# daducci/AMICO

Measured on AMD Instinct MI355X. Metric: voxels/sec (whole node), NODDI fit, higher is better.
Workload: dtype f64; 1 GPU; NODDI fit, 1000000 masked voxels per GPU, 99-volume 2-shell scheme (9 b0 + 30@b700 + 60@b2000), 145 atoms, ndirs=500, inputs resident in HBM; voxels_per_gpu=1000000, global_voxels=1000000, parallelism=voxel shards x1, one RCCL all_gather of the maps per step

## Files before the change

amico_amd/csrc/amx_kernels.hpp:

```cpp
#pragma once
#include <type_traits>
#include "amx_solver.hpp"
#include "amx_gram_solver.hpp"

namespace amx {

struct Chunk { int dir, start, count, pad; };
constexpr int kSeedKD = 12;
constexpr int kAuxU = 0, kAuxU2 = 12, kAuxB0 = 24, kAuxYY = 25, kAuxYB = 26, kAuxTmin = 27, kAuxN = 28;
__host__ __device__ constexpr int gemm_rows(int n_atoms) { return ((n_atoms + kAuxN + 15) / 16) * 16; }
constexpr int kScreenLd = 192;

enum StatusSlot { ST_ERRVOX = 0, ST_II1 = 1, ST_II2 = 2, ST_OVERFLOW = 3, ST_ITCAP = 4, ST_RERUN = 5, ST_GUARD = 6, ST_GUARDVOX = 7, ST_EXACT = 8, ST_GRAM = 11, ST_ITERS = 14, ST_SEED = 17, ST_LEFT = 92, ST_CLIP = 95, ST_ERRPACK = 96, ST_ERRKIND = 98, ST_WORDS = 100 };

struct FitCommon {
    const void *tiles;
    const double *y;
    const float *y32;
    const int *perm;
    const Chunk *chunks;
    const int *n_chunks;
    const int *list;
    const int *list_count;
    const int *lutidx;
// ... 208 lines not shown
        st_ = S.solve(As, ldA, nS, n_atoms, yr, rowok, scl, allowed, kLasso ? a.c.lam1 : 0.0, kLasso ? a.c.lam2 : 0.0, rs, rl, lane, gdir, a.ldG, seed, scr);
    }
    const int st = __builtin_amdgcn_readfirstlane(st_);
    if (st == kOverflow) {
        if (lane == 0) {
            const int k = atomicAdd(a.c.ovf_count, 1);
            a.c.ovf_list[k] = (STAGE == 4 && a.list_is_pos) ? pos : vox;
        }
    } else {
    if (st == kIterCap && lane == 0) atomicAdd(&a.c.status[ST_ITCAP], 1);
    if (st > kIterCap && lane == 0) { atomicAdd(&a.c.status[ST_GUARD], 1); a.c.status[ST_GUARDVOX] = vox * 8 + st; }
#ifdef AMX_PHASES
    if constexpr (STAGE == 1 || STAGE == 3) {
        if (lane == 0 && S.seeded == 1) {
            unsigned long long *acc = reinterpret_cast<unsigned long long *>(const_cast<int *>(a.c.n_chunks) + 16) + (STAGE == 1 ? 0 : 8);
            for (int k = 0; k < 8; k++) atomicAdd(&acc[k], (unsigned long long)S.ph[k]);
        }
    }
#endif
#ifdef AMX_STATS
    if (lane == 0) { constexpr int sx = kLasso ? 1 : STAGE - 1; atomicAdd(&a.c.status[ST_EXACT + sx], S.n_exact); atomicAdd(&a.c.status[ST_GRAM + sx], S.n_gram); atomicAdd(&a.c.status[ST_ITERS + sx], S.iters);
        if constexpr (STAGE == 4) { if (S.seeded >= 0) atomicAdd(&a.c.status[ST_SEED + 18], 1); if (S.seeded == 1) atomicAdd(&a.c.status[ST_SEED + 19], 1); }
        if constexpr (!kLasso) { if (S.seeded >= 0) atomicAdd(&a.c.status[ST_SEED + (STAGE == 1 ? 0 : 2)], 1); if (S.seeded == 1) atomicAdd(&a.c.status[ST_SEED + (STAGE == 1 ? 1 : 3)], 1); if (S.seeded == 0 && STAGE == 1) atomicAdd(&a.c.status[ST_SEED + 6 + S.seed_why], 1); } }
#endif
    const bool act = lane < S.np;
    if (a.c.xdbg) {
        constexpr int row = (STAGE == 1) ? 0 : (kLasso ? 1 : 2);
        double *dst = a.c.xdbg + ((size_t)vox * 3 + row) * n_atoms;
        store_x_dense<NQ>(dst, n_atoms, lane, S.np, S.idx, S.x);
        if (kLasso && lane == 0) {
            asm volatile("s_waitcnt vmcnt(0)" ::: "memory");
            dst[iso_atom] = a.xiso[(size_t)vox * 2];
            if (dot_atom >= 0) dst[dot_atom] = a.xiso[(size_t)vox * 2 + 1];
        }
    }

    if constexpr (STAGE == 1) {
        const unsigned long long mi = ballot64(act && S.idx == iso_atom), md = ballot64(act && S.idx == dot_atom);
        const double xi = mi ? bcast(S.x, __builtin_ctzll(mi)) : 0.0;
        const double xd = md ? bcast(S.x, __builtin_ctzll(md)) : 0.0;
        if (lane == 0) { a.xiso[(size_t)vox * 2] = xi; a.xiso[(size_t)vox * 2 + 1] = xd; }
    } else if constexpr (kLasso) {
        if (lane < 4) wmask[lane] = 0ull;
        if (act && S.x > 0.0) atomicOr(&wmask[S.idx >> 6], 1ull << (S.idx & 63));
        if (lane < 4) a.supp[(size_t)vox * 4 + lane] = wmask[lane];
    } else {
        double rsq = 0.0, ysq = 0.0;
        if (a.c.flags & 3u) {
            S.residual(yr, 0.0);
#pragma unroll
            for (int rr = 0; rr < NR; rr++) { rsq += S.r[rr] * S.r[rr]; ysq += yr[rr] * yr[rr]; }
            rsq = wave_sum(rsq); ysq = wave_sum(ysq);
        }
        const double xs = act ? S.x : 0.0;
        const bool iswm = act && S.idx < n_wm;
        const double sum_atoms = wave_sum(xs) + 1e-16;
        const double sum_wm = wave_sum(iswm ? xs / sum_atoms : 0.0) + 1e-16;
        double f1 = 0.0, f2 = 0.0, k1 = 0.0;
        if (iswm) {
            const float ic = a.icvf[S.idx];
            const double t = xs / sum_atoms / sum_wm;
            f1 = (double)ic * t;
            f2 = (double)((float)(1.0 - (double)ic)) * t;
            k1 = (double)a.kappa[S.idx] * t;
        }
        f1 = wave_sum(f1); f2 = wave_sum(f2); k1 = wave_sum(k1);
        const double ndi = f1 / (f1 + f2 + 1e-16);
        const double odi = odi_from_kappa(k1);
        const double fwf = wave_sum((act && S.idx == iso_atom) ? xs : 0.0) / sum_atoms;
        const double dot = wave_sum((act && S.idx == dot_atom) ? xs : 0.0) / sum_atoms;
        if (lane == 0) {
            double *e = a.est + (size_t)vox * a.n_maps;
            e[0] = ndi; e[1] = odi; e[2] = fwf;
            if (a.is_exvivo) e[3] = dot;
            if (a.rmse) a.rmse[vox] = sqrt(rsq / (double)nS);
            if (a.nrmse) a.nrmse[vox] = (ysq > 1e-16) ? sqrt(rsq / ysq) : 0.0;
            if (a.mod) { const double tf = 1.0 - fwf; a.mod[(size_t)vox * 2] = ndi * tf; a.mod[(size_t)vox * 2 + 1] = odi * tf; }
        }
    }
    }
    }
}

struct FwArgs {
    FitCommon c;
    int n_perp, n_iso, is_mouse, n_maps;
    double *est, *rmse, *nrmse, *ycorr;
    double *cproj;
    const double *prep;
    unsigned *p0;
    int ldC;
    int *queue;
    int sub_per_chunk;
};

template <int NR, int NQ, int MAXP>
__device__ __forceinline__ void fw_voxel(const FwArgs &a, const float *As, double *rs, double *rl, int vox, int lane)
{
    const int nS = a.c.nS, ldA = a.c.ldA, n_atoms = a.c.n_atoms, n_perp = a.n_perp;
    double yr[NR];
    const bool ok = load_rows<NR>(a.c, vox, nS, lane, yr);
    bool rowok[NR];
    double scl[NQ];
    unsigned long long allowed[NQ];
#pragma unroll
    for (int rr = 0; rr < NR; rr++) rowok[rr] = (lane + kWave * rr) < nS;
#pragma unroll
    for (int q = 0; q < NQ; q++) {
        const int cnt = n_atoms - kWave * q;
        allowed[q] = cnt >= 64 ? ~0ull : (cnt > 0 ? ((1ull << cnt) - 1ull) : 0ull);
        scl[q] = 1.0;
    }
    if (!ok) {
        if (lane < a.n_maps) a.est[(size_t)vox * a.n_maps + lane] = __builtin_nan("");
        if (lane == 0 && a.rmse) a.rmse[vox] = __builtin_nan("");
        if (lane == 0 && a.nrmse) a.nrmse[vox] = __builtin_nan("");
        if (a.ycorr)
            for (int i = lane; i < nS; i += kWave) a.ycorr[(size_t)vox * nS + i] = __builtin_nan("");
    }
    if (ok) {
    NNSolver<NR, NQ, MAXP, true, float> S;
    const int st = __builtin_amdgcn_readfirstlane(S.solve(As, ldA, nS, n_atoms, yr, rowok, scl, allowed, a.c.lam1, a.c.lam2, rs, rl, lane));
    if (st == kOverflow) {
        if (lane == 0) { const int k = atomicAdd(a.c.ovf_count, 1); a.c.ovf_list[k] = vox; }
    } else {
    if (st == kIterCap && lane == 0) atomicAdd(&a.c.status[ST_ITCAP], 1);
    if (st > kIterCap && lane == 0) { atomicAdd(&a.c.status[ST_GUARD], 1); a.c.status[ST_GUARDVOX] = vox * 8 + st; }
    const bool act = lane < S.np;
    const double xs = act ? S.x : 0.0;
    if (a.c.xdbg) store_x_dense<NQ>(a.c.xdbg + (size_t)vox * n_atoms, n_atoms, lane, S.np, S.idx, S.x);
    const double x_sum = wave_sum(xs) + 1e-16;
    const double v = wave_sum((act && S.idx < n_perp) ? xs : 0.0) / x_sum;
    const double vb = wave_sum((act && S.idx == n_perp) ? xs : 0.0) / x_sum;
    const double vc = wave_sum((act && S.idx == n_perp + 1) ? xs : 0.0) / x_sum;
    double rsq = 0.0, ysq = 0.0;
#pragma unroll
    for (int rr = 0; rr < NR; rr++) { rsq += S.r[rr] * S.r[rr]; ysq += yr[rr] * yr[rr]; }
    if (a.c.flags & 3u) { rsq = wave_sum(rsq); ysq = wave_sum(ysq); }
    if (lane == 0) {
        double *e = a.est + (size_t)vox * a.n_maps;
        e[0] = v; e[1] = 1.0 - v;
        if (a.is_mouse) { e[2] = vb; e[3] = vc; }
        if (a.rmse) a.rmse[vox] = sqrt(rsq / (double)nS);
        if (a.nrmse) a.nrmse[vox] = (ysq > 1e-16) ? sqrt(rsq / ysq) : 0.0;
    }
    if (a.ycorr) {
        double fw[NR];
#pragma unroll
        for (int rr = 0; rr < NR; rr++) fw[rr] = 0.0;
        for (int s = 0; s < S.np; s++) {
            const int at = bcast_i(S.idx, s);
            if (at >= n_perp) {
                const double xv = bcast(S.x, s);
#pragma unroll
                for (int rr = 0; rr < NR; rr++) {
                    const int i = lane + kWave * rr;
                    if (i < nS) fw[rr] += (double)As[i * ldA + at] * xv;
                }
            }
        }
#pragma unroll
        for (int rr = 0; rr < NR; rr++) {
            const int i = lane + kWave * rr;
            if (i < nS) { const double yc = yr[rr] - fw[rr]; a.ycorr[(size_t)vox * nS + i] = yc < 0.0 ? 0.0 : yc; }
        }
    }
// ... 105 lines not shown
    unsigned long long allowed[NQ];
#pragma unroll
    for (int rr = 0; rr < NR; rr++) rowok[rr] = (lane + kWave * rr) < nS;
#pragma unroll
    for (int q = 0; q < NQ; q++) {
        const int cnt = n_atoms - kWave * q;
        allowed[q] = cnt >= 64 ? ~0ull : (cnt > 0 ? ((1ull << cnt) - 1ull) : 0ull);
        scl[q] = 1.0;
    }
    if (!ok) {
        if (lane < 3) a.est[(size_t)vox * 3 + lane] = __builtin_nan("");
        if (lane == 0 && a.rmse) a.rmse[vox] = __builtin_nan("");
        if (lane == 0 && a.nrmse) a.nrmse[vox] = __builtin_nan("");
    }
    if (ok) {
    typename std::conditional<QR, NNSolver<NR, NQ, MAXP, true, float>, GramSolver<NR, NQ, MAXP, float>>::type S;
    const bool dense = NQ == 1 && n_atoms <= MAXP && a.c.lam2 >= 1e-2 && !(a.c.flags & 0x80000000u);
    int st_;
    if constexpr (QR) {
        st_ = S.solve(As, ldA, nS, n_atoms, yr, rowok, scl, allowed, a.c.lam1, a.c.lam2, rs, rl, lane);
    } else if constexpr (NQ == 1) {
        st_ = dense ? S.solve_dense(As, ldA, nS, n_atoms, yr, a.c.lam1, a.c.lam2, rs, rl, lane, gdir, a.ldG, Lf, lf_inv)
                    : S.solve(As, ldA, nS, n_atoms, yr, rowok, scl, allowed, a.c.lam1, a.c.lam2, rs, rl, lane, gdir, a.ldG);
    } else {
        st_ = S.solve(As, ldA, nS, n_atoms, yr, rowok, scl, allowed, a.c.lam1, a.c.lam2, rs, rl, lane, gdir, a.ldG);
    }
    const int st = __builtin_amdgcn_readfirstlane(st_);
    if (st == kOverflow) {
        if (lane == 0) { const int k = atomicAdd(a.c.ovf_count, 1); a.c.ovf_list[k] = vox; }
    } else {
    if (st == kIterCap && lane == 0) atomicAdd(&a.c.status[ST_ITCAP], 1);
    if (st > kIterCap && lane == 0) { atomicAdd(&a.c.status[ST_GUARD], 1); a.c.status[ST_GUARDVOX] = vox * 8 + st; }
    const bool act = lane < S.np;
    const int at = act ? S.idx : 0;
    const double xs = act ? S.x : 0.0;
    if (a.c.xdbg) store_x_dense<NQ>(a.c.xdbg + (size_t)vox * n_atoms, n_atoms, lane, S.np, S.idx, xs);
    double f1 = wave_sum((act && at < n_rs) ? xs : 0.0);
    const double f2 = wave_sum((act && at >= n_rs && at < n_rs + n_perp) ? xs : 0.0) + 1e-16;
    const double v = f1 / (f1 + f2 + 1e-16);
    f1 += 1e-16;
    double am = wave_sum((act && at < n_rs) ? a.Rs[at] * xs : 0.0);
    am = 1e6 * 2.0 * am / f1;
    const double d = (4.0 * v) / (3.14159265358979323846 * (am * am) + 1e-16);
    if (lane == 0) { double *e = a.est + (size_t)vox * 3; e[0] = v; e[1] = am; e[2] = d; }
    if (a.c.flags & 3u) {
        double est[NR];
#pragma unroll
        for (int rr = 0; rr < NR; rr++) est[rr] = 0.0;
        for (int s = 0; s < S.np; s++) {
            const int as = bcast_i(S.idx, s);
            const double xv = bcast(xs, s);
#pragma unroll
            for (int rr = 0; rr < NR; rr++) {
                const int i = lane + kWave * rr;
                if (i < nS) est[rr] += (double)As[i * ldA + as] * xv;
            }
        }
        double rsq = 0.0, ysq = 0.0;
#pragma unroll
        for (int rr = 0; rr < NR; rr++) { const double t = yr[rr] - est[rr]; rsq += t * t; ysq += yr[rr] * yr[rr]; }
        rsq = wave_sum(rsq); ysq = wave_sum(ysq);
        if (lane == 0) {
            if (a.rmse) a.rmse[vox] = sqrt(rsq / (double)nS);
            if (a.nrmse) a.nrmse[vox] = (ysq > 1e-16) ? sqrt(rsq / ysq) : 0.0;
        }
    }
    }
    }
}

__host__ __device__ constexpr int solver_lds_words(bool gram, int maxp, bool ridge = true)
{
    return gram ? (maxp + 1) * (maxp + 2) : (ridge ? 2 : 1) * (maxp + 1) * (maxp + 1);
}

__device__ __forceinline__ int xcd_chunk(int b, int n_chunks)
{
    const int per = (n_chunks + 7) >> 3;
    const int cid = (b & 7) * per + (b >> 3);
    return ((b >> 3) < per && cid < n_chunks) ? cid : -1;
}


__device__ __forceinline__ int next_ticket(unsigned *ticket, int lane)
{
    const unsigned off = (unsigned)(uintptr_t)ticket;
    const unsigned inc = lane == 0 ? 1u : 0u;
    unsigned old;
    asm volatile("ds_add_rtn_u32 %0, %1, %2\n\ts_waitcnt lgkmcnt(0)" : "=v"(old) : "v"(off), "v"(inc) : "memory");
    return __builtin_amdgcn_readfirstlane((int)old);
}

#define AMX_KERNEL_PROLOGUE_GT(AT, NRv, NQv, NWv, RLWv, GTv)                                                \
    extern __shared__ __attribute__((aligned(16))) unsigned char smem[];                              \
    const int lane = threadIdx.x & 63, wave = threadIdx.x >> 6;                                       \
    const int words = a.c.nS * a.c.ldA;                                                               \
    const int words_pad = (GTv) ? 0 : ((words + kWave * NQv + 3) & ~3);                               \
    AT *As = reinterpret_cast<AT *>(smem);                                                            \
    double *rs_all = reinterpret_cast<double *>(smem + (((size_t)words_pad * sizeof(AT) + 15) & ~(size_t)15)); \
    double *rs = rs_all + wave * (NRv * kWave);                                                       \
    const int nw_ = (int)blockDim.x >> 6;                     \
    double *rl_all = rs_all + nw_ * NRv * kWave;                                                      \
    double *rl = rl_all + wave * (RLWv);                                                              \
    unsigned long long *wm_all = reinterpret_cast<unsigned long long *>(rl_all + nw_ * (RLWv)); \
    unsigned long long *wmask = wm_all + wave * 4;                                                    \

#define AMX_KERNEL_PROLOGUE(AT, NRv, NQv, NWv, RLWv) AMX_KERNEL_PROLOGUE_GT(AT, NRv, NQv, NWv, RLWv, false)
constexpr int kTileSlack = 512;

template <int STAGE, int NR, int NQ, int MAXP, int NW, bool LIST, typename AT = float, bool GT = false>
__global__ void __launch_bounds__(NW * 64, (NW <= 4 && !LIST && !GT) ? 2 : 1) k_noddi(const NoddiArgs a)
{
    static_assert(!GT || std::is_same<AT, float>::value, "the global tile is the float32 dictionary itself");
    using ATs = typename std::conditional<GT, gtile<float>, AT>::type;
    constexpr int RLW = solver_lds_words(STAGE == 4, MAXP, STAGE == 2);
    AMX_KERNEL_PROLOGUE_GT(AT, NR, NQ, NW, RLW, GT)
    const float *tiles = reinterpret_cast<const float *>(a.c.tiles);
    if (!LIST) {
        const int cid = xcd_chunk((int)blockIdx.x, *a.c.n_chunks);
        if (cid < 0) return;
        const Chunk ck = a.c.chunks[cid];
        unsigned *ticket = reinterpret_cast<unsigned *>(wm_all + nw_ * 4);
        if ((STAGE == 1 || STAGE == 3 || STAGE == 4) && a.rlist != nullptr) {
            const int left = a.rcount[cid];
            if (left == 0) return;
            if (threadIdx.x == 0) atomicAdd(&a.c.status[ST_LEFT + (STAGE == 1 ? 0 : (STAGE == 3 ? 2 : 1))], left);
        }
        if (threadIdx.x == 0) { ticket[0] = (unsigned)nw_; ticket[1] = (unsigned)nw_; }
        const AT *At = As;
        if constexpr (GT) At = reinterpret_cast<const AT *>(tiles + (size_t)ck.dir * a.c.tile_stride);
        else stage_noddi_tile<AT>(As, tiles + (size_t)ck.dir * a.c.tile_stride, words, words_pad - words);
        float *Sf = nullptr;
        if ((STAGE == 1 || STAGE == 3) && a.scr_S != nullptr && a.seeds != nullptr) {
            Sf = reinterpret_cast<float *>(ticket + 4);
            const float *src = a.scr_S + (size_t)ck.dir * kSeedKD * kScreenLd;
            for (int e = threadIdx.x; e < kSeedKD * kScreenLd; e += blockDim.x) Sf[e] = src[e];
        }
        if (STAGE == 4 && a.scr2_S != nullptr && a.seeds2 != nullptr) {
            Sf = reinterpret_cast<float *>(ticket + 4);
            const float *src = a.scr2_S + (size_t)ck.dir * kSeedKD * kScreenLd;
            for (int e = threadIdx.x; e < kSeedKD * kScreenLd; e += blockDim.x) Sf[e] = src[e];
        }
        __syncthreads();
#ifdef AMX_STATIC_VOXELS
        for (int k = wave; k < ck.count; k += nw_) {
            noddi_voxel<STAGE, NR, NQ, MAXP, ATs>(a, reinterpret_cast<const ATs *>(At), rs, rl, wmask, a.c.perm[ck.start + k], ck.dir, lane);
        }
#else
        if ((STAGE == 1 || STAGE == 3 || STAGE == 4) && a.rlist != nullptr) {
            const int cnt = a.rcount[cid];
            const bool two = (STAGE == 1 || STAGE == 3) && a.done != nullptr;
            for (int pass = 0; pass < (two ? 2 : 1); pass++) {
                unsigned *tk = ticket + pass;
                for (int k = wave; k < cnt; k = next_ticket(tk, lane)) {
                    const int pos = a.rlist[ck.start + k];
                    if (two) {
                        const int flag = __builtin_amdgcn_readfirstlane((int)a.done[pos]);
                        if ((flag == 2) != (pass == 1)) continue;
                    }
                    noddi_voxel<STAGE, NR, NQ, MAXP, ATs>(a, reinterpret_cast<const ATs *>(At), rs, rl, wmask, a.c.perm[pos], ck.dir, lane, pos, Sf);
                }
            }
        } else {
            for (int k = wave; k < ck.count; k = next_ticket(ticket, lane)) {
                noddi_voxel<STAGE, NR, NQ, MAXP, ATs>(a, reinterpret_cast<const ATs *>(At), rs, rl, wmask, a.c.perm[ck.start + k], ck.dir, lane, ck.start + k, Sf);
            }
        }
#endif
    } else {
        const int cnt = *a.c.list_count;
        for (int it = blockIdx.x; it < cnt; it += gridDim.x) {
            const int e = a.c.list[it];
            const int pos = (STAGE == 4 && a.list_is_pos) ? e : -1;
            const int vox = (STAGE == 4 && a.list_is_pos) ? a.c.perm[e] : e;
            if constexpr (GT) {
                noddi_voxel<STAGE, NR, NQ, MAXP, ATs>(a, reinterpret_cast<const ATs *>(tiles + (size_t)a.c.lutidx[vox] * a.c.tile_stride), rs, rl, wmask, vox, a.c.lutidx[vox], lane, pos);
            } else {
                __syncthreads();
                stage_noddi_tile<AT>(As, tiles + (size_t)a.c.lutidx[vox] * a.c.tile_stride, words, words_pad - words);
                __syncthreads();
                noddi_voxel<STAGE, NR, NQ, MAXP, AT>(a, As, rs, rl, wmask, vox, a.c.lutidx[vox], lane, pos);
            }
        }
    }
}

template <int NR, int NQ, int MAXP, int NW, bool LIST>
__global__ void __launch_bounds__(NW * 64) k_freewater(const FwArgs a)
{
    AMX_KERNEL_PROLOGUE(float, NR, NQ, NW, solver_lds_words(false, MAXP))
    (void)wmask;
    const float *tiles = reinterpret_cast<const float *>(a.c.tiles);
    if (!LIST) {
        const int cid = xcd_chunk((int)blockIdx.x, *a.c.n_chunks);
        if (cid < 0) return;
        const Chunk ck = a.c.chunks[cid];
        unsigned *ticket = reinterpret_cast<unsigned *>(wm_all + nw_ * 4);
        if (threadIdx.x == 0) *ticket = (unsigned)nw_;
        stage_tile<float>(As, tiles + (size_t)ck.dir * a.c.tile_stride, words, words_pad - words);
        __syncthreads();
        for (int k = wave; k < ck.count; k = next_ticket(ticket, lane)) {
            fw_voxel<NR, NQ, MAXP>(a, As, rs, rl, a.c.perm[ck.start + k], lane);
        }
    } else {
        const int cnt = *a.c.list_count;
        for (int it = blockIdx.x; it < cnt; it += gridDim.x) {
            const int vox = a.c.list[it];
            __syncthreads();
            stage_tile<float>(As, tiles + (size_t)a.c.lutidx[vox] * a.c.tile_stride, words, words_pad - words);
            __syncthreads();
            fw_voxel<NR, NQ, MAXP>(a, As, rs, rl, vox, lane);
        }
    }
}

template <int NR, int NQ, int MAXP, int NW, bool LIST>
__global__ void __launch_bounds__(NW * 64) k_sandi(const SandiArgs a)
{
    AMX_KERNEL_PROLOGUE(double, NR, NQ, NW, solver_lds_words(false, MAXP))
    (void)wmask;
    const double *tiles = reinterpret_cast<const double *>(a.c.tiles);
    if (!LIST) {
        const int cid = xcd_chunk((int)blockIdx.x, *a.c.n_chunks);
        if (cid < 0) return;
        const Chunk ck = a.c.chunks[cid];
        unsigned *ticket = reinterpret_cast<unsigned *>(wm_all + nw_ * 4);
        if (threadIdx.x == 0) *ticket = (unsigned)nw_;
        stage_tile<double>(As, tiles, words, words_pad - words);
        __syncthreads();
        for (int k = wave; k < ck.count; k = next_ticket(ticket, lane)) {
            sandi_voxel<NR, NQ, MAXP>(a, As, rs, rl, a.c.perm[ck.start + k], lane);
        }
    } else {
        const int cnt = *a.c.list_count;
        stage_tile<double>(As, tiles, words, words_pad - words);
        __syncthreads();
// ... 169 lines not shown
```

amico_amd/csrc/amx_solver.hpp:

```cpp
#pragma once
#include <hip/hip_runtime.h>
#include <stdint.h>

namespace amx {

constexpr int kWave = 64;

#ifdef AMX_PHASES
#define AMX_PH(k) do { const long long t__ = (long long)__builtin_readcyclecounter(); ph[k] += t__ - pht; pht = t__; } while (0)
#else
#define AMX_PH(k) do { } while (0)
#endif
enum SolveStatus : int { kSolved = 0, kOverflow = 1, kIterCap = 2, kGuardSelect = 3, kGuardOuter = 4 };
struct SeedScreen {
    const float *Sf = nullptr;
    int ld = 0;
    double kappa = 0.0;
    const double *ytil = nullptr;
    const double *Sg = nullptr;
    int *count = nullptr;
};
constexpr unsigned long long kSeedNone = ~0ull;

__device__ __forceinline__ double bcast(double v, int l)
{
    int lo = __builtin_amdgcn_readlane(__double2loint(v), l);
    int hi = __builtin_amdgcn_readlane(__double2hiint(v), l);
    return __hiloint2double(hi, lo);
}
__device__ __forceinline__ int bcast_i(int v, int l) { return __builtin_amdgcn_readlane(v, l); }

template <int CTRL, int ROWM, int BANKM>
__device__ __forceinline__ double dpp_move(double v, double ident)
{
    int lo = __builtin_amdgcn_update_dpp(__double2loint(ident), __double2loint(v), CTRL, ROWM, BANKM, false);
    int hi = __builtin_amdgcn_update_dpp(__double2hiint(ident), __double2hiint(v), CTRL, ROWM, BANKM, false);
    return __hiloint2double(hi, lo);
}
template <int CTRL>
__device__ __forceinline__ double dpp_zero(double v)
{
    int lo = __builtin_amdgcn_update_dpp(0, __double2loint(v), CTRL, 0xf, 0xf, true);
    int hi = __builtin_amdgcn_update_dpp(0, __double2hiint(v), CTRL, 0xf, 0xf, true);
    return __hiloint2double(hi, lo);
}
#define AMX_ROW_SWAP(BUILTIN, k, A, B)                                                                             \
    do {                                                                                                           \
        const auto lo_ = BUILTIN((unsigned)__double2loint(k), (unsigned)__double2loint(k), false, false);          \
        const auto hi_ = BUILTIN((unsigned)__double2hiint(k), (unsigned)__double2hiint(k), false, false);          \
        A = __hiloint2double((int)hi_[0], (int)lo_[0]); B = __hiloint2double((int)hi_[1], (int)lo_[1]);            \
    } while (0)
__device__ __forceinline__ double rows_allreduce(double k)
{
    double a, b;
    AMX_ROW_SWAP(__builtin_amdgcn_permlane16_swap, k, a, b); k = a + b;
    AMX_ROW_SWAP(__builtin_amdgcn_permlane32_swap, k, a, b); k = a + b;
    return k;
}
__device__ __forceinline__ double wave_sum(double v)
{
    double t = v + dpp_zero<0xB1>(v);
    t += dpp_zero<0x4E>(t);
    t += dpp_zero<0x141>(t);
    t += dpp_zero<0x140>(t);
    return rows_allreduce(t);
}
__device__ __forceinline__ double wave_max(double v)
{
    double t = fmax(v, dpp_zero<0xB1>(v));
    t = fmax(t, dpp_zero<0x4E>(t));
    t = fmax(t, dpp_zero<0x141>(t));
    t = fmax(t, dpp_zero<0x140>(t));
    double a, b;
    AMX_ROW_SWAP(__builtin_amdgcn_permlane16_swap, t, a, b); t = fmax(a, b);
    AMX_ROW_SWAP(__builtin_amdgcn_permlane32_swap, t, a, b); t = fmax(a, b);
    return t;
}
__device__ __forceinline__ double wave_min(double v) { return -wave_max(-v); }
__device__ __forceinline__ double rows_allmax(double k)
{
    double a, b;
    AMX_ROW_SWAP(__builtin_amdgcn_permlane16_swap, k, a, b); k = fmax(a, b);
    AMX_ROW_SWAP(__builtin_amdgcn_permlane32_swap, k, a, b); k = fmax(a, b);
    return k;
}
// ... 722 lines not shown
                } else {
                    AMX_PH(3);
                    const int kn = np;
#pragma unroll
                    for (int m = 0; m < MAXP; m++) {
                        if (m == kn) {
#pragma unroll
                            for (int rr = 0; rr < NR; rr++) Q[m][rr] = v[rr] * binv;
                        }
                    }
                    if (lane <= kn) Rl[lane * LDR + kn] = (lane == kn) ? beta : rho;
                    if (RIDGE && lane <= kn) Ql[lane * LDR + kn] = va * binv;
                    if (lane == kn) { d = dnew; e = enew; rinv = binv; x = 0.0; sc = sct; idx = t; }
                    fl &= 0xff00ffffu; cyc_banned = false;
                    if (lane == tl) fl |= 0x100u << tq;
                    np = kn + 1;
                    last_added = t;
                    added = true;

                }
            }
            if (redo) continue;
            if (!added) {
                if (status == kSolved && cyc_banned && second_looks < 3) {
                    fl &= 0xff00ffffu; cyc_banned = false; second_looks++; force_exact = true; last_added = -1;
                    continue;
                }
                break;
            }

            AMX_PH(4);
            for (bool feasible = false; !feasible && status == kSolved;) {
                if (++iters > itmax) { status = kIterCap; break; }
                double rhs = d - lam1 * e;
                {
                    const int li = (lane < MAXP ? lane : MAXP - 1) * LDR;
                    for (int j = np - 1; j >= 0; j--) {
                        const double col = Rl[li + j];
                        const double zj = bcast(rhs * rinv, j);
                        if (lane < j) rhs -= col * zj;
                    }
                }
                const double z = (lane < np) ? rhs * rinv : 0.0;
                const bool act = lane < np;
                const bool neg = act && !(z > 0.0);
                AMX_PH(5);
                const bool any = ballot64(neg) != 0ull;
                unsigned long long rem = 0ull;
                if (any) {
                    const double den = x - z;
                    const double ratio = neg ? ((den > 0.0) ? x / den : 0.0) : inf;
                    const double alpha = wave_min(ratio);
                    const unsigned long long hit = ballot64(neg && ratio == alpha);
                    const int kmin = hit ? __builtin_ctzll(hit) : -1;
                    x = act ? x + alpha * (z - x) : 0.0;
                    if (lane == kmin) x = 0.0;
                    rem = ballot64(act && !(x > 0.0));
                } else {
                    x = act ? z : 0.0;
                }
                for (int guard = 0; rem != 0ull && guard < kWave; ++guard) {
                    const int k = 63 - __builtin_clzll(rem);
                    rem &= ~(1ull << k);
                    const int a = bcast_i(idx, k);
                    if (a == last_added) { cyc_banned = true; if (lane == (a & 63)) fl |= 0x10000u << (a >> 6); }
                    if (G != nullptr) {
                        const double dl = -bcast(sc * xprev, k);
                        const double *gc = G + (size_t)a * ldG + lane;
#pragma unroll
                        for (int q = 0; q < NQ; q++) u[q] -= gc[kWave * q] * dl;
                    }
                    if (lane == (a & 63)) fl &= ~(0x1000000u << (a >> 6));
                    remove_slot(k, lane, fl);
                }
                if (np == 0) x = 0.0;
                feasible = !any || np == 0;
                AMX_PH(6);
            }
        }
        return status;
    }
};

}
```

Baseline: 156.0 million voxels/s.

## Certify seeded NNLS voxels four per wave using 16-lane groups

Adds a group-level certification path for the second pass of NNLS stages 1 and 3. Voxels whose seed marks them as likely solvable are processed four per wavefront, one per 16-lane group. Each group verifies the seeded active set with a small Cholesky solve plus KKT screening using DPP group reductions. Voxels that fail certification fall back to the full per-wave solver, so wasted certification work and extra register pressure are the risk.

```diff
diff --git a/amico_amd/csrc/amx_kernels.hpp b/amico_amd/csrc/amx_kernels.hpp
--- a/amico_amd/csrc/amx_kernels.hpp
+++ b/amico_amd/csrc/amx_kernels.hpp
@@ -314,6 +314,106 @@
     }
 }
 
+template <int STAGE, int NRG, int NQG, typename AT>
+__device__ __forceinline__ bool noddi_group_voxel(const NoddiArgs &a, const AT *As, int pos, int dir, int lane, const float *Sf)
+{
+    static_assert(STAGE == 1 || STAGE == 3, "NNLS stages only");
+    const int nS = a.c.nS, ldA = a.c.ldA, n_atoms = a.c.n_atoms, n_wm = a.n_wm;
+    const int iso_atom = n_atoms - 1, dot_atom = a.is_exvivo ? n_atoms - 2 : -1;
+    const int g = lane & (kGroup - 1);
+    const bool have = pos >= 0;
+    const int vox = have ? a.c.perm[pos] : 0;
+    double yr[NRG];
+    bool finite = true;
+#pragma unroll
+    for (int rr = 0; rr < NRG; rr++) {
+        const int i = g + kGroup * rr;
+        yr[rr] = 0.0;
+        if (have && i < nS) yr[rr] = (a.c.y32 != nullptr) ? (double)a.c.y32[(size_t)vox * nS + i] : a.c.y[(size_t)vox * nS + i];
+        finite = finite && (fabs(yr[rr]) <= 1.79769313486231570e308);
+    }
+    bool go = have && gballot(!finite, lane) == 0u;
+    unsigned long long allowed[4] = {0ull, 0ull, 0ull, 0ull};
+#pragma unroll
+    for (int q = 0; q < 4; q++) {
+        const int cnt = n_atoms - 64 * q;
+        allowed[q] = cnt >= 64 ? ~0ull : (cnt > 0 ? ((1ull << cnt) - 1ull) : 0ull);
+    }
+    if (STAGE == 3 && go) {
+#pragma unroll
+        for (int q = 0; q < 4; q++) allowed[q] &= a.supp[(size_t)vox * 4 + q];
+        allowed[iso_atom >> 6] |= 1ull << (iso_atom & 63);
+        if (dot_atom >= 0) allowed[dot_atom >> 6] |= 1ull << (dot_atom & 63);
+    }
+    const unsigned long long seed = go ? a.seeds[pos] : kSeedNone;
+    go = go && seed != kSeedNone;
+    SeedScreen scr;
+    scr.Sf = Sf; scr.ld = kScreenLd; scr.kappa = a.scr_kappa[dir];
+    scr.ytil = a.scr_ytil + (size_t)(go ? pos : 0) * kSeedKD; scr.Sg = a.scr_Sg + (size_t)dir * n_atoms * kSeedKD;
+    GroupCert<NRG, NQG, AT> S;
+    const double *gdir = a.gram + (size_t)dir * n_atoms * a.ldG;
+    if (ballot64(go) == 0ull) return false;
+    go = S.certify(As, ldA, nS, yr, allowed, go ? seed : 0ull, gdir, a.ldG, scr, lane, go);
+    if (ballot64(go) == 0ull) return false;
+    if (go) {
+        const bool act = g < S.np;
+#ifdef AMX_STATS
+        if (g == 0) {
+            atomicAdd(&a.c.status[ST_EXACT + STAGE - 1], 1);
+            atomicAdd(&a.c.status[ST_SEED + (STAGE == 1 ? 0 : 2)], 1); atomicAdd(&a.c.status[ST_SEED + (STAGE == 1 ? 1 : 3)], 1);
+        }
+#endif
+        if (a.c.xdbg) {
+            double *dst = a.c.xdbg + ((size_t)vox * 3 + (STAGE == 1 ? 0 : 2)) * n_atoms;
+#pragma unroll
+            for (int q = 0; q < NQG; q++) {
+                const int j = g + kGroup * q;
+                if (j < n_atoms) dst[j] = 0.0;
+            }
+            asm volatile("s_waitcnt vmcnt(0)" ::: "memory");
+            if (act) dst[S.idx] = S.x;
+        }
+        if constexpr (STAGE == 1) {
+            const unsigned mi = gballot(act && S.idx == iso_atom, lane), md = gballot(act && S.idx == dot_atom, lane);
+            const double xi = gbcast_dyn(S.x, mi ? __builtin_ctz(mi) : 0, lane), xd = gbcast_dyn(S.x, md ? __builtin_ctz(md) : 0, lane);
+            if (g == 0) { a.xiso[(size_t)vox * 2] = mi ? xi : 0.0; a.xiso[(size_t)vox * 2 + 1] = md ? xd : 0.0; }
+        } else {
+            double rsq = 0.0, ysq = 0.0;
+            if (a.c.flags & 3u) {
+#pragma unroll
+                for (int rr = 0; rr < NRG; rr++) rsq += S.r[rr] * S.r[rr];
+                rsq = gsum(rsq); ysq = S.ysq;
+            }
+            const double xs = act ? S.x : 0.0;
+            const bool iswm = act && S.idx < n_wm;
+            const double sum_atoms = gsum(xs) + 1e-16;
+            const double sum_wm = gsum(iswm ? xs / sum_atoms : 0.0) + 1e-16;
+            double f1 = 0.0, f2 = 0.0, k1 = 0.0;
+            if (iswm) {
+                const float ic = a.icvf[S.idx];
+                const double t = xs / sum_atoms / sum_wm;
+                f1 = (double)ic * t;
+                f2 = (double)((float)(1.0 - (double)ic)) * t;
+                k1 = (double)a.kappa[S.idx] * t;
+            }
+            f1 = gsum(f1); f2 = gsum(f2); k1 = gsum(k1);
+            const double ndi = f1 / (f1 + f2 + 1e-16);
+            const double odi = odi_from_kappa(k1);
+            const double fwf = gsum((act && S.idx == iso_atom) ? xs : 0.0) / sum_atoms;
+            const double dot = gsum((act && S.idx == dot_atom) ? xs : 0.0) / sum_atoms;
+            if (g == 0) {
+                double *e = a.est + (size_t)vox * a.n_maps;
+                e[0] = ndi; e[1] = odi; e[2] = fwf;
+                if (a.is_exvivo) e[3] = dot;
+                if (a.rmse) a.rmse[vox] = sqrt(rsq / (double)nS);
+                if (a.nrmse) a.nrmse[vox] = (ysq > 1e-16) ? sqrt(rsq / ysq) : 0.0;
+                if (a.mod) { const double tf = 1.0 - fwf; a.mod[(size_t)vox * 2] = ndi * tf; a.mod[(size_t)vox * 2 + 1] = odi * tf; }
+            }
+        }
+    }
+    return go;
+}
+
 struct FwArgs {
     FitCommon c;
     int n_perp, n_iso, is_mouse, n_maps;
@@ -585,10 +685,10 @@
 }
 
 
-__device__ __forceinline__ int next_ticket(unsigned *ticket, int lane)
+__device__ __forceinline__ int next_ticket(unsigned *ticket, int lane, unsigned step = 1u)
 {
     const unsigned off = (unsigned)(uintptr_t)ticket;
-    const unsigned inc = lane == 0 ? 1u : 0u;
+    const unsigned inc = lane == 0 ? step : 0u;
     unsigned old;
     asm volatile("ds_add_rtn_u32 %0, %1, %2\n\ts_waitcnt lgkmcnt(0)" : "=v"(old) : "v"(off), "v"(inc) : "memory");
     return __builtin_amdgcn_readfirstlane((int)old);
@@ -629,7 +729,7 @@
             if (left == 0) return;
             if (threadIdx.x == 0) atomicAdd(&a.c.status[ST_LEFT + (STAGE == 1 ? 0 : (STAGE == 3 ? 2 : 1))], left);
         }
-        if (threadIdx.x == 0) { ticket[0] = (unsigned)nw_; ticket[1] = (unsigned)nw_; }
+        if (threadIdx.x == 0) { ticket[0] = (unsigned)nw_; ticket[1] = (unsigned)nw_; ticket[2] = 4u * (unsigned)nw_; }
         const AT *At = As;
         if constexpr (GT) At = reinterpret_cast<const AT *>(tiles + (size_t)ck.dir * a.c.tile_stride);
         else stage_noddi_tile<AT>(As, tiles + (size_t)ck.dir * a.c.tile_stride, words, words_pad - words);
@@ -653,8 +753,30 @@
         if ((STAGE == 1 || STAGE == 3 || STAGE == 4) && a.rlist != nullptr) {
             const int cnt = a.rcount[cid];
             const bool two = (STAGE == 1 || STAGE == 3) && a.done != nullptr;
+            constexpr bool kGroupShape = (STAGE == 1 || STAGE == 3) && !GT && NR == 2;
+            const bool groups = kGroupShape && two && Sf != nullptr && a.gram != nullptr && a.seeds != nullptr;
             for (int pass = 0; pass < (two ? 2 : 1); pass++) {
                 unsigned *tk = ticket + pass;
+                if constexpr (kGroupShape) {
+                    if (pass == 1 && groups) {
+                        for (int kb = 4 * wave; kb < cnt; kb = next_ticket(ticket + 2, lane, 4u)) {
+                            const int k = kb + (lane >> 4);
+                            int pos = -1;
+                            if (k < cnt) {
+                                const int p = a.rlist[ck.start + k];
+                                if (a.done[p] == 2) pos = p;
+                            }
+                            const bool fin = noddi_group_voxel<STAGE, 4 * NR, 4 * NQ, ATs>(a, reinterpret_cast<const ATs *>(At), pos, ck.dir, lane, Sf);
+                            for (unsigned long long rest = ballot64(pos >= 0 && !fin); rest != 0ull;) {
+                                const int l = __builtin_ctzll(rest);
+                                rest &= ~(0xffffull << l);
+                                const int p = __builtin_amdgcn_readlane(pos, l);
+                                noddi_voxel<STAGE, NR, NQ, MAXP, ATs>(a, reinterpret_cast<const ATs *>(At), rs, rl, wmask, a.c.perm[p], ck.dir, lane, p, Sf);
+                            }
+                        }
+                        continue;
+                    }
+                }
                 for (int k = wave; k < cnt; k = next_ticket(tk, lane)) {
                     const int pos = a.rlist[ck.start + k];
                     if (two) {
diff --git a/amico_amd/csrc/amx_solver.hpp b/amico_amd/csrc/amx_solver.hpp
--- a/amico_amd/csrc/amx_solver.hpp
+++ b/amico_amd/csrc/amx_solver.hpp
@@ -1,6 +1,8 @@
 #pragma once
 #include <hip/hip_runtime.h>
 #include <stdint.h>
+#include <type_traits>
+#include <utility>
 
 namespace amx {
 
@@ -889,4 +891,265 @@
     }
 };
 
-}
+constexpr int kGroup = 16;
+template <typename F, int... I>
+__device__ __forceinline__ void sfor_(F &&f, std::integer_sequence<int, I...>) { (f(std::integral_constant<int, I>{}), ...); }
+template <int N, typename F>
+__device__ __forceinline__ void sfor(F &&f) { sfor_(f, std::make_integer_sequence<int, N>{}); }
+
+__device__ __forceinline__ double gsum(double v)
+{
+    double t = v + dpp_zero<0xB1>(v);
+    t += dpp_zero<0x4E>(t);
+    t += dpp_zero<0x141>(t);
+    return t + dpp_zero<0x140>(t);
+}
+__device__ __forceinline__ double gmax(double v)
+{
+    double t = fmax(v, dpp_zero<0xB1>(v));
+    t = fmax(t, dpp_zero<0x4E>(t));
+    t = fmax(t, dpp_zero<0x141>(t));
+    return fmax(t, dpp_zero<0x140>(t));
+}
+template <int K>
+__device__ __forceinline__ double gbcast(double v) { return dpp_zero<0x150 + K>(v); }
+template <int K>
+__device__ __forceinline__ int gbcast_i(int v) { return __builtin_amdgcn_update_dpp(0, v, 0x150 + K, 0xf, 0xf, true); }
+__device__ __forceinline__ double gbcast_dyn(double v, int k, int lane)
+{
+    const int addr = ((lane & ~(kGroup - 1)) + k) * 4;
+    const int lo = __builtin_amdgcn_ds_bpermute(addr, __double2loint(v));
+    const int hi = __builtin_amdgcn_ds_bpermute(addr, __double2hiint(v));
+    return __hiloint2double(hi, lo);
+}
+__device__ __forceinline__ int gbcast_dyn_i(int v, int k, int lane)
+{
+    return __builtin_amdgcn_ds_bpermute(((lane & ~(kGroup - 1)) + k) * 4, v);
+}
+__device__ __forceinline__ unsigned gballot(bool p, int lane) { return (unsigned)(ballot64(p) >> (lane & 48)) & 0xffffu; }
+
+template <int NRG, int NQG, typename AT>
+struct GroupCert {
+    static constexpr int MAXS = 8;
+    double r[NRG];
+    double ysq;
+    double x;
+    int idx;
+    int np;
+    int lane_, npw_;
+
+    __device__ __forceinline__ void column(const AT *As, int ldA, int nS, int t, int g, double (&col)[NRG]) const
+    {
+        AT raw[NRG] = {};
+#pragma unroll
+        for (int rr = 0; rr < NRG; rr++) {
+            const int i = g + kGroup * rr;
+            if (i < nS) raw[rr] = As[i * ldA + t];
+        }
+#pragma unroll
+        for (int rr = 0; rr < NRG; rr++) col[rr] = (g + kGroup * rr < nS) ? (double)raw[rr] : 0.0;
+    }
+    __device__ __forceinline__ double slot_dots(const AT *As, int ldA, int nS, const double (&v)[NRG], int g) const
+    {
+        double out = 0.0;
+#pragma unroll 1
+        for (int m = 0; m < npw_; m++) {
+            const int t = (m < np) ? gbcast_dyn_i(idx, m, lane_) : 0;
+            double col[NRG];
+            column(As, ldA, nS, t, g, col);
+            double p = 0.0;
+#pragma unroll
+            for (int rr = 0; rr < NRG; rr++) p += col[rr] * v[rr];
+            p = gsum(p);
+            if (g == m && m < np) out = p;
+        }
+        return out;
+    }
+    __device__ __forceinline__ void sub_cols(const AT *As, int ldA, int nS, double c, int g, double (&v)[NRG]) const
+    {
+#pragma unroll 1
+        for (int m = 0; m < npw_; m++) {
+            const int t = (m < np) ? gbcast_dyn_i(idx, m, lane_) : 0;
+            const double cm = (m < np) ? gbcast_dyn(c, m, lane_) : 0.0;
+            double col[NRG];
+            column(As, ldA, nS, t, g, col);
+#pragma unroll
+            for (int rr = 0; rr < NRG; rr++) v[rr] -= col[rr] * cm;
+        }
+    }
+    __device__ __forceinline__ double chol_solve(double rhs, const double (&Lr)[MAXS], const double (&Lc)[MAXS], double rinv, int g) const
+    {
+        double f = (g < np) ? rhs : 0.0;
+        sfor<MAXS>([&](auto kc) {
+            constexpr int k = decltype(kc)::value;
+            const double wk = gbcast<k>(f * rinv);
+            if (k < np && g > k) f -= Lr[k] * wk;
+        });
+        double b = f * rinv;
+        sfor<MAXS>([&](auto kc) {
+            constexpr int k = MAXS - 1 - decltype(kc)::value;
+            const double zk = gbcast<k>(b * rinv);
+            if (k < np && g < k) b -= Lc[k] * zk;
+        });
+        return (g < np) ? b * rinv : 0.0;
+    }
+
+    __device__ __forceinline__ bool certify(const AT *As, int ldA, int nS, const double (&yr)[NRG], const unsigned long long (&allowed)[4],
+                                            unsigned long long seed, const double *__restrict__ G, int ldG, const SeedScreen &scr, int lane, bool go)
+    {
+        constexpr int KDs = 12;
+        const int g = lane & (kGroup - 1);
+        lane_ = lane;
+        const int my = (int)((seed >> (8 * (g & 7))) & 0xffull);
+        const unsigned present = gballot(g < MAXS && my < 0xf0, lane);
+        const int n0 = __builtin_popcount(present);
+        bool ok = go && present == ((1u << n0) - 1u) && n0 > 0;
+        np = ok ? n0 : 0;
+        idx = (g < np) ? my : -1;
+        {
+            const bool adm = idx >= 0 && idx < kGroup * NQG && ((allowed[(idx >> 6) & 3] >> (idx & 63)) & 1ull);
+            bool bad = g < np && !adm;
+            sfor<MAXS>([&](auto sc) {
+                constexpr int s = decltype(sc)::value;
+                const int t = gbcast_i<s>(idx);
+                if (g > s && g < np && idx == t) bad = true;
+            });
+            ok = ok && gballot(bad, lane) == 0u;
+        }
+        if (!ok) np = 0;
+        npw_ = __builtin_amdgcn_readfirstlane((int)wave_max((double)np));
+        ysq = 0.0;
+#pragma unroll
+        for (int rr = 0; rr < NRG; rr++) { r[rr] = yr[rr]; ysq += yr[rr] * yr[rr]; }
+        ysq = gsum(ysq);
+        x = 0.0;
+        double Lr[MAXS], Lc[MAXS];
+        sfor<MAXS>([&](auto kc) {
+            constexpr int k = decltype(kc)::value;
+            const int tk = gbcast_i<k>(idx);
+            Lr[k] = 0.0;
+            if (k < np && g >= k && g < np) Lr[k] = G[(size_t)idx * ldG + tk];
+        });
+        const double c0 = slot_dots(As, ldA, nS, yr, g);
+        double rinv = 0.0;
+        sfor<MAXS>([&](auto kc) {
+            constexpr int k = decltype(kc)::value;
+            if (k < np) {
+                double t = Lr[k];
+                const double hkk = gbcast<k>(t);
+#pragma unroll
+                for (int m = 0; m < k; m++) t -= Lr[m] * gbcast<k>(Lr[m]);
+                const double tk = gbcast<k>(t);
+                ok = ok && tk > 1e-14 * hkk;
+                const double iv = inv_sqrt(tk > 0.0 ? tk : 1.0);
+                if (g >= k && g < np) Lr[k] = t * iv;
+                if (g == k) rinv = iv;
+            }
+        });
+        sfor<MAXS>([&](auto kc) {
+            constexpr int k = decltype(kc)::value;
+            Lc[k] = 0.0;
+#pragma unroll
+            for (int i = 0; i < k; i++) {
+                const double v = gbcast<k>(Lr[i]);
+                if (g == i) Lc[k] = v;
+            }
+        });
+        if (ok) {
+            x = chol_solve(c0, Lr, Lc, rinv, g);
+            sub_cols(As, ldA, nS, x, g, r);
+            bool live = true;
+            double gprev = __builtin_huge_val();
+            for (int it = 0; it < 5; it++) {
+                if (ballot64(live) == 0ull) break;
+                if (live) {
+                    const double gr = slot_dots(As, ldA, nS, r, g);
+                    const double gm = gmax((g < np) ? fabs(gr) : 0.0);
+                    if (gm < 2e-15) {
+                        live = false;
+                    } else if (!(gm < 0.25 * gprev)) {
+                        live = false; ok = gm < 1e-12;
+                    } else {
+                        gprev = gm;
+                        const double dx = chol_solve(gr, Lr, Lc, rinv, g);
+                        x += dx;
+                        sub_cols(As, ldA, nS, dx, g, r);
+                        if (it == 4) { live = false; ok = false; }
+                    }
+                }
+            }
+            ok = ok && gballot(g < np && !(x > 0.0), lane) == 0u;
+        }
+        if (ballot64(ok) == 0ull) return false;
+        if (ok) {
+            unsigned out = 0u;
+#pragma unroll
+            for (int q = 0; q < NQG; q++) {
+                const int j = g + kGroup * q;
+                if ((allowed[j >> 6] >> (j & 63)) & 1ull) out |= 1u << q;
+            }
+            sfor<MAXS>([&](auto sc) {
+                constexpr int s = decltype(sc)::value;
+                const int t = gbcast_i<s>(idx);
+                if (s < np && g == (t & (kGroup - 1))) out &= ~(1u << (t >> 4));
+            });
+            double rsq = 0.0;
+#pragma unroll
+            for (int rr = 0; rr < NRG; rr++) rsq += r[rr] * r[rr];
+            rsq = gsum(rsq);
+            const bool zero_res = rsq <= 1e-28 * ysq;
+            if (zero_res) out = 0u;
+            const bool direct = gsum((double)__builtin_popcount(out)) <= 12.0;
+            float ut[NQG];
+#pragma unroll
+            for (int q = 0; q < NQG; q++) ut[q] = 0.0f;
+            if (!direct) {
+                const int l12 = g < KDs ? g : 0;
+                double rt = scr.ytil[l12];
+                double sv[MAXS];
+                sfor<MAXS>([&](auto mc) {
+                    constexpr int m = decltype(mc)::value;
+                    const int t = gbcast_i<m>(idx);
+                    sv[m] = scr.Sg[(size_t)(m < np ? t : 0) * KDs + l12];
+                });
+                rt = (g < KDs) ? rt : 0.0;
+                sfor<MAXS>([&](auto mc) {
+                    constexpr int m = decltype(mc)::value;
+                    const double xs = gbcast<m>(x);
+                    if (m < np && g < KDs) rt -= sv[m] * xs;
+                });
+#pragma unroll 1
+                for (int dd = 0; dd < KDs; dd++) {
+                    const float rd = (float)gbcast_dyn(rt, dd, lane);
+#pragma unroll
+                    for (int q = 0; q < NQG; q++) ut[q] += scr.Sf[dd * scr.ld + g + kGroup * q] * rd;
+                }
+            }
+            const float margin = direct ? __builtin_huge_valf() : (float)(1.0625 * scr.kappa * sqrt(rsq));
+            unsigned todo = 0u;
+#pragma unroll
+            for (int q = 0; q < NQG; q++) if (((out >> q) & 1u) && !(ut[q] < -margin)) todo |= 1u << q;
+            bool viol = false;
+            for (int guard = 0; guard < kGroup * NQG; guard++) {
+                const double mine = todo ? (double)(g + kGroup * __builtin_ctz(todo)) : 1e9;
+                const double tmin = -gmax(-mine);
+                if (ballot64(tmin < 1e9) == 0ull) break;
+                const bool has = tmin < 1e9;
+                const int t = has ? (int)tmin : 0;
+                if (has && g == (t & (kGroup - 1))) todo &= ~(1u << (t >> 4));
+                double col[NRG];
+                column(As, ldA, nS, t, g, col);
+                double p = 0.0;
+#pragma unroll
+                for (int rr = 0; rr < NRG; rr++) p += col[rr] * r[rr];
+                p = gsum(p);
+                viol = viol || (has && p > 0.0);
+            }
+            ok = !viol;
+        }
+        if (!ok) { np = 0; idx = -1; x = 0.0; }
+        return ok;
+    }
+};
+
+}
```

Measured after the change: 150.1 million voxels/s, median of 2. -3.8%, worse.
